# DigITs-AIML/MMNN_STS

Measured on AMD Instinct MI355X. Metric: training volumes/sec/GPU (128^3 T1+T2+preop, batch 2) at 1/2/4/8 MI355X, higher is better.
Workload: dtype f32; 1 GPU; configs[2] --images --preop --survival --blend: MultiModalModel(DenseNet121-3D(in=2), MLP(32), blend) fwd + GradientBlender Cox loss + bwd + grad all-reduce + SGD-Nesterov/OneCycle step, dropout 0.2; micro_batch=2, global_batch=2, tabular=32, parallelism=dp1, allreduce=none

## Files before the change

### mmnn_sts_amd/csrc/conv3_bf16x3.hip

```cpp
#include <stdlib.h>

#include "fprop.hpp"
#include "bf16x3.hpp"

namespace mmnn {

typedef float f32x16_t __attribute__((ext_vector_type(16)));
typedef __bf16 bf16x8_t __attribute__((ext_vector_type(8)));

namespace c3b {
constexpr int KC = 16, NT = 7, MAXC = 256;
template <int TD, int TH, int TW>
struct Geo {
  static constexpr int HD = TD + 2, HH = TH + 2, HW = TW + 2, HV = HD * HH * HW, ROWS = TD * TH * TW / 32;
  static constexpr int ITEMS = (2 * HV + 255) / 256;
  static constexpr size_t OPER_BYTES = (size_t)2 * 6 * HV * 16;
  static constexpr size_t SMEM = OPER_BYTES + sizeof(float) * (2 * 4 * 32 + 32);
  static_assert(TD * TH * TW % 32 == 0 && (TW == 32 || TW == 16), "rows of 32 voxels");
  static_assert(ITEMS <= NT, "one staging item per tap slot");
  static_assert(4 * ROWS * 16 * 64 * sizeof(float) <= OPER_BYTES, "the partial tiles are summed in the operand buffers");
  static_assert(SMEM <= 160 * 1024, "LDS");
};

__device__ __forceinline__ bf16x8_t as_bf16x8(uint4 v) { return __builtin_bit_cast(bf16x8_t, v); }
}

__global__ void __launch_bounds__(256) conv3_split_bnrelu_kernel(const FpropArgs a) {
  __shared__ float cf[2][8];
  const int c8 = blockIdx.y, n = blockIdx.z, C8 = a.Cin / 8, V = a.D * a.H * a.W;
  const int v = blockIdx.x * 256 + threadIdx.x;
  const float* __restrict__ x = a.in0 + (long)n * a.in0_ns + (long)(a.in0_coff + 8 * c8) * V;
  float xv[8];
#pragma unroll
  for (int e = 0; e < 8; ++e) xv[e] = v < V ? x[(long)e * V + v] : 0.f;
  if (threadIdx.x < 8) {
    float ca, cb, mu, rs;
    bn_fwd_coef(a.bn_in, 8 * c8 + threadIdx.x, ca, cb, mu, rs);
    cf[0][threadIdx.x] = ca; cf[1][threadIdx.x] = cb;
  }
  __syncthreads();
  if (v >= V) return;
#pragma unroll
  for (int e = 0; e < 8; ++e) xv[e] = fmaxf(fmaf(cf[0][e], xv[e], cf[1][e]), 0.f);
  uint4 hi, mid, lo;
  split3x8(xv, hi, mid, lo);
  const long ps = (long)a.N * C8 * V;
  uint4* __restrict__ dst = reinterpret_cast<uint4*>(a.x3) + ((long)n * C8 + c8) * V + v;
  dst[0] = hi; dst[ps] = mid; dst[2 * ps] = lo;
}

__global__ void __launch_bounds__(256) conv3_split_bnbwd_kernel(const FpropArgs a) {
  __shared__ float cf[3][8];
  const int c8 = blockIdx.y, n = blockIdx.z, C8 = a.Cin / 8, V = a.D * a.H * a.W;
  const int v = blockIdx.x * 256 + threadIdx.x;
  const float* __restrict__ gn = a.in0 + (long)n * a.in0_ns + (long)(a.in0_coff + 8 * c8) * V;
  const float* __restrict__ xn = a.in1 + (long)n * a.in1_ns + (long)(a.in1_coff + 8 * c8) * V;
  float gv[8], xv[8];
#pragma unroll
  for (int e = 0; e < 8; ++e) {
    gv[e] = v < V ? gn[(long)e * V + v] : 0.f;
    xv[e] = v < V ? xn[(long)e * V + v] : 0.f;
  }
  if (threadIdx.x < 8) {
    const int c = 8 * c8 + threadIdx.x;
    float p_, q_, r_;
    bn_bwd_coef(a.gr_in, c, p_, q_, r_);
    const float sc = drop_scale(a.drop_in, n, c);
    cf[0][threadIdx.x] = p_ * sc; cf[1][threadIdx.x] = q_ * sc; cf[2][threadIdx.x] = r_ * sc;
  }
  __syncthreads();
  if (v >= V) return;
#pragma unroll
  for (int e = 0; e < 8; ++e) gv[e] = fmaf(cf[0][e], gv[e], fmaf(cf[1][e], xv[e], cf[2][e]));
  uint4 hi, mid, lo;
  split3x8(gv, hi, mid, lo);
  const long ps = (long)a.N * C8 * V;
  uint4* __restrict__ dst = reinterpret_cast<uint4*>(a.x3) + ((long)n * C8 + c8) * V + v;
  dst[0] = hi; dst[ps] = mid; dst[2 * ps] = lo;
}

static int launch_split(bool bwd, const FpropArgs& a, hipStream_t stream) {
  const int V = a.D * a.H * a.W;
  const dim3 grid((unsigned)cdiv(V, 256), (unsigned)(a.Cin / 8), (unsigned)a.N);
  if (bwd) MMNN_LAUNCH(conv3_split_bnbwd_kernel, grid, dim3(256), 0, stream, a);
  else MMNN_LAUNCH(conv3_split_bnrelu_kernel, grid, dim3(256), 0, stream, a);
  MMNN_HIP(hipGetLastError());
  return 0;
}

template <int TD, int TH, int TW>
__global__ void __launch_bounds__(256) conv3_fwd_bf16x3_kernel(const FpropArgs a) {
  using namespace c3b;
  using G = Geo<TD, TH, TW>;
  constexpr int HH = G::HH, HW = G::HW, HV = G::HV, ROWS = G::ROWS, ITEMS = G::ITEMS;
  constexpr size_t OPER_BYTES = G::OPER_BYTES;
  extern __shared__ uint4 xs128[];
  float* const sred = reinterpret_cast<float*>(reinterpret_cast<char*>(xs128) + OPER_BYTES);
  float* const dsc = sred + 2 * 4 * 32;
  const int tid = threadIdx.x, lane = tid & 63, wv = tid >> 6;
  const int D = a.D, H = a.H, W = a.W, V = D * H * W, C8 = a.Cin / 8, nchunk = a.Cin / KC;
  const int twn = (W + TW - 1) / TW, thn = (H + TH - 1) / TH, tdn = (D + TD - 1) / TD;
  int b = blockIdx.x;
  const int w0 = (b % twn) * TW; b /= twn;
  const int h0 = (b % thn) * TH; b /= thn;
  const int d0 = (b % tdn) * TD;
  const int n = b / tdn;
  const long ps = (long)a.N * C8 * V;
  const uint4* __restrict__ xin = reinterpret_cast<const uint4*>(a.x3) + (long)n * C8 * V;
  const uint4* __restrict__ wp = reinterpret_cast<const uint4*>(a.w3);
  if (tid < 32) dsc[tid] = drop_scale(a.drop_out, n, tid);
  f32x16_t acc[ROWS];
#pragma unroll
  for (int t = 0; t < ROWS; ++t)
#pragma unroll
    for (int q = 0; q < 16; ++q) acc[t][q] = 0.f;
  uint4 xr[ITEMS][3];
  auto item_pos = [&](int it, int& g, int& hv, int& o) -> bool {
    const int item = tid + it * 256;
    g = item >= HV;
    hv = item - g * HV;
    const int hd = hv / (HH * HW), hh = (hv / HW) % HH, hw = hv % HW;
    const int d = d0 + hd - 1, h = h0 + hh - 1, w = w0 + hw - 1;
    o = (d * H + h) * W + w;
    return item < 2 * HV && (unsigned)d < (unsigned)D && (unsigned)h < (unsigned)H && (unsigned)w < (unsigned)W;
  };
  auto issue = [&](int ch) {
#pragma unroll
    for (int it = 0; it < ITEMS; ++it) {
      int g, hv, o;
      const bool ok = item_pos(it, g, hv, o);
      const uint4* src = xin + (long)(2 * ch + g) * V + o;
#pragma unroll
      for (int p = 0; p < 3; ++p) xr[it][p] = ok ? src[p * ps] : make_uint4(0u, 0u, 0u, 0u);
    }
  };
  auto commit_item = [&](int it, int buf) {
    int g, hv, o;
    item_pos(it, g, hv, o);
    if (tid + it * 256 >= 2 * HV) return;
    uint4* dst = xs128 + buf * (6 * HV);
#pragma unroll
    for (int p = 0; p < 3; ++p) dst[(p * 2 + g) * HV + hv] = xr[it][p];
  };
  bf16x8_t wr[NT][3];
  auto load_w = [&](int ti, int ch) {
    const int tap = wv + 4 * ti;
    if (tap < 27 && ch < nchunk) {
      const int c8 = 2 * ch + (lane >> 5);
#pragma unroll
      for (int p = 0; p < 3; ++p) wr[ti][p] = as_bf16x8(wp[((long)(p * 27 + tap) * C8 + c8) * 32 + (lane & 31)]);
    }
  };
#pragma unroll
  for (int ti = 0; ti < NT; ++ti) load_w(ti, 0);
  issue(0);
#pragma unroll
  for (int it = 0; it < ITEMS; ++it) commit_item(it, 0);
  __syncthreads();
  for (int ch = 0; ch < nchunk; ++ch) {
    const int cur = ch & 1;
    const bool more = ch + 1 < nchunk;
    if (more) issue(ch + 1);
#pragma unroll
    for (int ti = 0; ti < NT; ++ti) {
      const int tap = wv + 4 * ti;
      if (tap < 27) {
        const int td = tap / 9, th = (tap / 3) % 3, tw = tap % 3;
        bf16x8_t aw[3];
#pragma unroll
        for (int p = 0; p < 3; ++p) aw[p] = wr[ti][p];
        load_w(ti, ch + 1);
#pragma unroll
        for (int t = 0; t < ROWS; ++t) {
          const int v = t * 32 + (lane & 31);
          const int hv = ((v / (TW * TH) + td) * HH + ((v / TW) % TH + th)) * HW + (v % TW + tw);
          bf16x8_t bb[3];
#pragma unroll
          for (int p = 0; p < 3; ++p) bb[p] = as_bf16x8(xs128[cur * (6 * HV) + (p * 2 + (lane >> 5)) * HV + hv]);
          acc[t] = __builtin_amdgcn_mfma_f32_32x32x16_bf16(aw[1], bb[1], acc[t], 0, 0, 0);
          acc[t] = __builtin_amdgcn_mfma_f32_32x32x16_bf16(aw[0], bb[2], acc[t], 0, 0, 0);
          acc[t] = __builtin_amdgcn_mfma_f32_32x32x16_bf16(aw[2], bb[0], acc[t], 0, 0, 0);
          acc[t] = __builtin_amdgcn_mfma_f32_32x32x16_bf16(aw[0], bb[1], acc[t], 0, 0, 0);
          acc[t] = __builtin_amdgcn_mfma_f32_32x32x16_bf16(aw[1], bb[0], acc[t], 0, 0, 0);
          acc[t] = __builtin_amdgcn_mfma_f32_32x32x16_bf16(aw[0], bb[0], acc[t], 0, 0, 0);
        }
      }
      if (more && ti < ITEMS) commit_item(ti, cur ^ 1);
    }
    __syncthreads();
  }
  float* red = reinterpret_cast<float*>(xs128);
#pragma unroll
  for (int t = 0; t < ROWS; ++t)
#pragma unroll
    for (int q = 0; q < 16; ++q) red[((wv * ROWS + t) * 16 + q) * 64 + lane] = acc[t][q];
  __syncthreads();
  float* __restrict__ outn = a.out + (long)n * a.out_ns + (long)a.out_coff * V;
  const bool want_sums = a.st_out.sum != nullptr;
  float s0[16], s1[16];
#pragma unroll
  for (int q = 0; q < 16; ++q) { s0[q] = 0.f; s1[q] = 0.f; }
#pragma unroll
  for (int tt = 0; tt < (ROWS + 3) / 4; ++tt) {
    const int t = wv + 4 * tt;
    if (t >= ROWS) break;
    const int v = t * 32 + (lane & 31);
    const int d = d0 + v / (TW * TH), h = h0 + (v / TW) % TH, w = w0 + v % TW;
    const bool ok = d < D && h < H && w < W;
    const int o = (d * H + h) * W + w;
#pragma unroll
    for (int q = 0; q < 16; ++q) {
      float val = 0.f;
#pragma unroll
      for (int w2 = 0; w2 < 4; ++w2) val += red[((w2 * ROWS + t) * 16 + q) * 64 + lane];
      const int m = 8 * (q / 4) + 4 * (lane >> 5) + q % 4;
      val *= dsc[m];
      if (ok) {
        outn[(long)m * V + o] = val;
        s0[q] += val;
        s1[q] += val * val;
      }
    }
  }
  if (want_sums) {
#pragma unroll
    for (int q = 0; q < 16; ++q) {
      float t0 = s0[q], t1 = s1[q];
      t0 += swz_xor<16>(t0); t1 += swz_xor<16>(t1);
      t0 += swz_xor<8>(t0);  t1 += swz_xor<8>(t1);
      t0 += swz_xor<4>(t0);  t1 += swz_xor<4>(t1);
      t0 += swz_xor<2>(t0);  t1 += swz_xor<2>(t1);
      t0 += swz_xor<1>(t0);  t1 += swz_xor<1>(t1);
      if ((lane & 31) == 0) {
        const int m = 8 * (q / 4) + 4 * (lane >> 5) + q % 4;
        sred[wv * 32 + m] = t0;
        sred[4 * 32 + wv * 32 + m] = t1;
      }
    }
    __syncthreads();
    if (tid < 32) {
      const int rep = blockIdx.x & ((a.nrep > 0 ? a.nrep : NREP) - 1);
      double v0 = 0.0, v1 = 0.0;
#pragma unroll
      for (int w2 = 0; w2 < 4; ++w2) { v0 += (double)sred[w2 * 32 + tid]; v1 += (double)sred[4 * 32 + w2 * 32 + tid]; }
      atomicAdd(a.st_out.sum + (long)rep * a.st_out.stride + a.st_out.off + tid, v0);
      atomicAdd(a.st_out.sq + (long)rep * a.st_out.stride + a.st_out.off + tid, v1);
    }
  }
}

__global__ void __launch_bounds__(256) conv3_dgrad_bf16x3_kernel(const FpropArgs a) {
  using namespace c3b;
  using G = Geo<2, 4, 32>;
  constexpr int TH = 4, TW = 32, HH = G::HH, HW = G::HW, HV = G::HV, ROWS = G::ROWS, ITEMS = G::ITEMS, PF = 3, C8 = 4;
  extern __shared__ uint4 xs128[];
  float* const ecoef = reinterpret_cast<float*>(reinterpret_cast<char*>(xs128) + G::OPER_BYTES);
  const int tid = threadIdx.x, lane = tid & 63, wv = tid >> 6;
  const int D = a.D, H = a.H, W = a.W, V = D * H * W;
  const int twn = (W + TW - 1) / TW, thn = (H + TH - 1) / TH, tdn = (D + 1) / 2;
  int b = blockIdx.x;
  const int w0 = (b % twn) * TW; b /= twn;
  const int h0 = (b % thn) * TH; b /= thn;
  const int d0 = (b % tdn) * 2;
  const int n = b / tdn;
  const long ps = (long)a.N * C8 * V;
  const uint4* __restrict__ xin = reinterpret_cast<const uint4*>(a.x3) + (long)n * C8 * V;
  const uint4* __restrict__ wp = reinterpret_cast<const uint4*>(a.w3);
  uint4 xr[ITEMS][3];
  auto item_pos = [&](int it, int& g, int& hv, int& o) -> bool {
    const int item = tid + it * 256;
    g = item >= HV;
    hv = item - g * HV;
    const int hd = hv / (HH * HW), hh = (hv / HW) % HH, hw = hv % HW;
    const int d = d0 + hd - 1, h = h0 + hh - 1, w = w0 + hw - 1;
    o = (d * H + h) * W + w;
    return item < 2 * HV && (unsigned)d < (unsigned)D && (unsigned)h < (unsigned)H && (unsigned)w < (unsigned)W;
  };
  auto issue = [&](int ch) {
#pragma unroll
    for (int it = 0; it < ITEMS; ++it) {
      int g, hv, o;
      const bool ok = item_pos(it, g, hv, o);
      const uint4* src = xin + (long)(2 * ch + g) * V + o;
#pragma unroll
      for (int p = 0; p < 3; ++p) xr[it][p] = ok ? src[p * ps] : make_uint4(0u, 0u, 0u, 0u);
    }
  };
  auto commit = [&](int buf) {
#pragma unroll
    for (int it = 0; it < ITEMS; ++it) {
      int g, hv, o;
      item_pos(it, g, hv, o);
      if (tid + it * 256 < 2 * HV) {
        uint4* dst = xs128 + buf * (6 * HV);
#pragma unroll
        for (int p = 0; p < 3; ++p) dst[(p * 2 + g) * HV + hv] = xr[it][p];
      }
    }
  };
  bf16x8_t wr[PF][3];
  auto load_w = [&](int slot, int tap, int ch) {
    if (ch < 2) {
      const int c8 = 2 * ch + (lane >> 5);
#pragma unroll
      for (int p = 0; p < 3; ++p) wr[slot][p] = as_bf16x8(wp[((long)(p * 27 + tap) * C8 + c8) * 128 + wv * 32 + (lane & 31)]);
    }
  };
#pragma unroll
  for (int t = 0; t < PF; ++t) load_w(t, t, 0);
  issue(0);
  if (tid >= 128) {
    const int m = tid - 128;
    float ea, eb, mu, rs;
    bn_fwd_coef(a.ebn, m, ea, eb, mu, rs);
    ecoef[m] = ea; ecoef[128 + m] = eb; ecoef[256 + m] = mu; ecoef[384 + m] = rs;
  }
  commit(0);
  issue(1);
  __syncthreads();
  f32x16_t acc[ROWS];
#pragma unroll
  for (int t = 0; t < ROWS; ++t)
#pragma unroll
    for (int q = 0; q < 16; ++q) acc[t][q] = 0.f;
  auto pair = [&](int ch, int tq) {
    const int td = tq / 3, th = tq % 3;
#pragma unroll
    for (int tw = 0; tw < 3; ++tw) {
      const int tap = tq * 3 + tw;
      bf16x8_t aw[3];
#pragma unroll
      for (int p = 0; p < 3; ++p) aw[p] = wr[tw][p];
      if (tq < 8) load_w(tw, tap + PF, ch); else load_w(tw, tw, ch + 1);
#pragma unroll
      for (int t = 0; t < ROWS; ++t) {
        const int hv = ((t / TH + td) * HH + (t % TH + th)) * HW + ((lane & 31) + tw);
        bf16x8_t bb[3];
#pragma unroll
        for (int p = 0; p < 3; ++p) bb[p] = as_bf16x8(xs128[ch * (6 * HV) + (p * 2 + (lane >> 5)) * HV + hv]);
        acc[t] = __builtin_amdgcn_mfma_f32_32x32x16_bf16(aw[1], bb[1], acc[t], 0, 0, 0);
        acc[t] = __builtin_amdgcn_mfma_f32_32x32x16_bf16(aw[0], bb[2], acc[t], 0, 0, 0);
        acc[t] = __builtin_amdgcn_mfma_f32_32x32x16_bf16(aw[2], bb[0], acc[t], 0, 0, 0);
        acc[t] = __builtin_amdgcn_mfma_f32_32x32x16_bf16(aw[0], bb[1], acc[t], 0, 0, 0);
        acc[t] = __builtin_amdgcn_mfma_f32_32x32x16_bf16(aw[1], bb[0], acc[t], 0, 0, 0);
        acc[t] = __builtin_amdgcn_mfma_f32_32x32x16_bf16(aw[0], bb[0], acc[t], 0, 0, 0);
      }
    }
  };
  pair(0, 0);
  commit(1);
  __syncthreads();
#pragma unroll 1
  for (int tq = 1; tq < 9; ++tq) pair(0, tq);
#pragma unroll 1
  for (int tq = 0; tq < 9; ++tq) pair(1, tq);
  const float* __restrict__ exn = a.ex + (long)n * a.ex_ns + (long)a.ex_coff * V;
  float* __restrict__ outn = a.out + (long)n * a.out_ns + (long)a.out_coff * V;
  float s0[16], s1[16];
#pragma unroll
  for (int q = 0; q < 16; ++q) { s0[q] = 0.f; s1[q] = 0.f; }
  auto row_pos = [&](int t, int& o) -> bool {
    const int d = d0 + t / TH, h = h0 + t % TH, w = w0 + (lane & 31);
    o = (d * H + h) * W + w;
    return d < D && h < H && w < W;
  };
  float xn[16];
  {
    int o;
    const bool ok = row_pos(0, o);
#pragma unroll
    for (int q = 0; q < 16; ++q) xn[q] = ok ? exn[(long)(wv * 32 + 8 * (q / 4) + 4 * (lane >> 5) + q % 4) * V + o] : 0.f;
  }
#pragma unroll
  for (int t = 0; t < ROWS; ++t) {
    int o;
    const bool ok = row_pos(t, o);
    float xe[16];
#pragma unroll
    for (int q = 0; q < 16; ++q) xe[q] = xn[q];
    if (t + 1 < ROWS) {
      int o2;
      const bool ok2 = row_pos(t + 1, o2);
#pragma unroll
      for (int q = 0; q < 16; ++q) xn[q] = ok2 ? exn[(long)(wv * 32 + 8 * (q / 4) + 4 * (lane >> 5) + q % 4) * V + o2] : 0.f;
    }
#pragma unroll
    for (int q = 0; q < 16; ++q) {
      const int m = wv * 32 + 8 * (q / 4) + 4 * (lane >> 5) + q % 4;
      if (ok) {
        const float pre = fmaf(ecoef[m], xe[q], ecoef[128 + m]);
        const float z = pre > 0.f ? acc[t][q] : 0.f;
        const float xh = (xe[q] - ecoef[256 + m]) * ecoef[384 + m];
        outn[(long)m * V + o] = z;
        s0[q] += z;
        s1[q] += z * xh;
      }
    }
  }
  const int rep = blockIdx.x & ((a.nrep > 0 ? a.nrep : NREP) - 1);
#pragma unroll
  for (int q = 0; q < 16; ++q) {
    float t0 = s0[q], t1 = s1[q];
    t0 += swz_xor<16>(t0); t1 += swz_xor<16>(t1);
    t0 += swz_xor<8>(t0);  t1 += swz_xor<8>(t1);
    t0 += swz_xor<4>(t0);  t1 += swz_xor<4>(t1);
    t0 += swz_xor<2>(t0);  t1 += swz_xor<2>(t1);
    t0 += swz_xor<1>(t0);  t1 += swz_xor<1>(t1);
    if ((lane & 31) == 0) {
      const int m = wv * 32 + 8 * (q / 4) + 4 * (lane >> 5) + q % 4;
      atomicAdd(a.dbeta + (long)rep * a.M + m, (double)t0);
      atomicAdd(a.dgamma + (long)rep * a.M + m, (double)t1);
    }
  }
}

size_t conv3_bf16x3_plane_bytes(const FpropArgs& a) { return (size_t)3 * a.N * (a.Cin / 8) * a.D * a.H * a.W * 16; }

bool conv3_dgrad_bf16x3_eligible(const FpropArgs& a) {
  static const int mode = [] { const char* e = getenv("MMNN_BF16X3_DGRAD"); return e ? atoi(e) : 1; }();
  static const int fmode = [] { const char* e = getenv("MMNN_BF16X3"); return e ? atoi(e) : 32; }();
  return mode != 0 && fmode != 0 && a.M == 128 && a.Cin == 32 && a.W > 16;
}

int launch_conv3_dgrad_bf16x3(const FpropArgs& a, hipStream_t stream) {
  using G = c3b::Geo<2, 4, 32>;
  constexpr size_t SMEM = G::OPER_BYTES + sizeof(float) * 512;
  static_assert(SMEM <= 160 * 1024, "LDS");
  MMNN_REQUIRE(conv3_dgrad_bf16x3_eligible(a), "conv3 dgrad bf16x3: shape not handled (M=%d, Cin=%d, W=%d)", a.M, a.Cin, a.W);
  MMNN_REQUIRE(a.in1 && a.ex && a.dgamma && a.dbeta, "conv3 dgrad bf16x3: operands missing");
  MMNN_REQUIRE(a.w3 && a.x3 && a.x3_bytes >= conv3_bf16x3_plane_bytes(a), "conv3 dgrad bf16x3: pre-split weights or plane scratch missing");
  MMNN_REQUIRE((long)(a.M + 1) * a.D * a.H * a.W < (1l << 31), "conv3 dgrad bf16x3: volume too large for 32-bit element offsets");
  const long tiles = (long)a.N * cdiv(a.D, 2) * cdiv(a.H, 4) * cdiv(a.W, 32);
  MMNN_REQUIRE(tiles > 0 && tiles < (1l << 31), "conv3 dgrad bf16x3: grid out of range");
  static bool configured[MAX_DEVICES] = {false};
  bool& conf = configured[current_device_slot()];
  if (!conf) {
    MMNN_HIP(hipFuncSetAttribute(reinterpret_cast<const void*>(conv3_dgrad_bf16x3_kernel), hipFuncAttributeMaxDynamicSharedMemorySize, (int)SMEM));
    conf = true;
  }
  if (int rc = launch_split(true, a, stream)) return rc;
  MMNN_LAUNCH(conv3_dgrad_bf16x3_kernel, dim3((unsigned)tiles), dim3(256), SMEM, stream, a);
  MMNN_HIP(hipGetLastError());
  return 0;
}

bool conv3_fwd_bf16x3_eligible(const FpropArgs& a) {
  static const int mode = [] { const char* e = getenv("MMNN_BF16X3"); return e ? atoi(e) : 32; }();
  return mode != 0 && a.M == 32 && a.Cin % c3b::KC == 0 && a.Cin >= c3b::KC && a.Cin <= c3b::MAXC && a.W > 16;
}

int launch_conv3_fwd_bf16x3(const FpropArgs& a, hipStream_t stream) {
  using G = c3b::Geo<2, 4, 32>;
  MMNN_REQUIRE(conv3_fwd_bf16x3_eligible(a), "conv3 bf16x3: shape not handled (M=%d, Cin=%d, W=%d)", a.M, a.Cin, a.W);
  MMNN_REQUIRE(a.drop_in.p <= 0.f, "conv3 bf16x3: no input dropout on this path");
  MMNN_REQUIRE(a.w3 && a.x3 && a.x3_bytes >= conv3_bf16x3_plane_bytes(a), "conv3 bf16x3: pre-split weights or plane scratch missing");
  MMNN_REQUIRE((long)(a.Cin + 1) * a.D * a.H * a.W < (1l << 31), "conv3 bf16x3: volume too large for 32-bit element offsets");
  const long tiles = (long)a.N * cdiv(a.D, 2) * cdiv(a.H, 4) * cdiv(a.W, 32);
  MMNN_REQUIRE(tiles > 0 && tiles < (1l << 31), "conv3 bf16x3: grid out of range");
  static bool configured[MAX_DEVICES] = {false};
  bool& conf = configured[current_device_slot()];
  if (!conf) {
    MMNN_HIP(hipFuncSetAttribute(reinterpret_cast<const void*>(conv3_fwd_bf16x3_kernel<2, 4, 32>), hipFuncAttributeMaxDynamicSharedMemorySize, (int)G::SMEM));
    conf = true;
  }
  if (int rc = launch_split(false, a, stream)) return rc;
  MMNN_LAUNCH((conv3_fwd_bf16x3_kernel<2, 4, 32>), dim3((unsigned)tiles), dim3(256), G::SMEM, stream, a);
  MMNN_HIP(hipGetLastError());
  return 0;
}

}
```

### mmnn_sts_amd/csrc/densenet.hip

```cpp
#include "densenet.hpp"

#include <string.h>

#include <algorithm>

#include "fprop.hpp"
#include "stem.hpp"
#include "wgrad.hpp"

namespace mmnn {

static size_t align_up(size_t v, size_t a = 256) { return (v + a - 1) / a * a; }
constexpr size_t KZ_PART_BYTES = (size_t)512 * 4 * 1024 * sizeof(float);
constexpr unsigned KZ_CNT_ENTRIES = 4096;

namespace {
struct Panel { const float* p; unsigned bytes; };
struct Carver {
  size_t cur = 0;
  size_t take(size_t bytes) {
    size_t o = cur;
    cur = align_up(cur + bytes);
    return o;
  }
// ... 55 lines not shown
      bn(p.mid, lo.n2w, lo.n2b, lo.r2m, lo.r2v);
      lo.c2 = po; po += conv2_elems(p);
      p.layers[b].push_back(lo);
      ci += cfg.growth;
    }
    if (b != cfg.nblocks - 1) {
      TransOff t;
      t.cin = ci; t.cout = ci / 2;
      bn(ci, t.nw, t.nb, t.rm, t.rv);
      t.cw = po; po += trans_elems(t);
      p.trans.push_back(t);
    } else {
      bn(ci, p.p_n5w, p.p_n5b, p.r_n5m, p.r_n5v);
    }
  }
  p.n_params = po; p.n_runstats = ro; p.n_bn = nbn;

  Carver cv;
  const int nb = cfg.nblocks;
  const size_t F = sizeof(float);
  const long V0 = (long)p.D0 * p.H0 * p.W0;
  p.o_conv0 = cv.take((size_t)N * cfg.init_features * V0 * F);
  p.o_idx = cv.take((size_t)N * cfg.init_features * p.Vb[0]);
  p.o_t1.assign(nb, {});
  size_t dap = 0;
  for (int b = 0; b < nb; ++b) {
    p.o_x[b] = cv.take((size_t)N * p.ctot_b[b] * p.Vb[b] * F);
    p.o_g[b] = cv.take((size_t)N * p.ctot_b[b] * p.Vb[b] * F);
    for (int l = 0; l < cfg.block_layers[b]; ++l) p.o_t1[b].push_back(cv.take((size_t)N * p.mid * p.Vb[b] * F));
    if (b != nb - 1) {
      p.o_ap[b] = cv.take((size_t)N * p.ctot_b[b] * p.Vb[b + 1] * F);
      dap = std::max(dap, (size_t)N * p.ctot_b[b] * p.Vb[b + 1] * F);
    } else {
      p.o_ap[b] = 0;
    }
  }
  p.o_dap = cv.take(dap ? dap : 256);
  p.o_dz0 = cv.take((size_t)N * cfg.init_features * V0 * F);
  const size_t PAIR = 2 * NREP * sizeof(double);
  p.o_fstat = cv.cur;
  p.o_st_conv0 = cv.take(PAIR * cfg.init_features);
  p.o_st_t1.assign(nb, {});
  for (int b = 0; b < nb; ++b) {
    p.o_st_x[b] = cv.take(PAIR * p.ctot_b[b]);
    for (int l = 0; l < cfg.block_layers[b]; ++l) p.o_st_t1[b].push_back(cv.take(PAIR * p.mid));
  }
  p.fstat_bytes = cv.cur - p.o_fstat;
  p.o_bstat = cv.cur;
  p.o_dg_n0 = cv.take(PAIR * cfg.init_features);
  p.o_dg_n1.assign(nb, {}); p.o_dg_n2.assign(nb, {}); p.o_dg_tr.clear();
  for (int b = 0; b < nb; ++b) {
    p.o_s_x[b] = cv.take(PAIR * p.ctot_b[b]);
    for (int l = 0; l < cfg.block_layers[b]; ++l) {
      p.o_dg_n1[b].push_back(cv.take(PAIR * p.layers[b][l].cin));
      p.o_dg_n2[b].push_back(cv.take(PAIR * p.mid));
    }
    if (b != nb - 1) p.o_dg_tr.push_back(cv.take(PAIR * p.ctot_b[b]));
  }
  p.o_dg_n5 = cv.take(PAIR * p.ctot_b[nb - 1]);
  p.bstat_bytes = cv.cur - p.o_bstat;
  p.o_pk_conv0 = cv.take((size_t)7 * stem_krows(cfg.in_channels) * 64 * F);
  p.o_pk_c1.assign(nb, {}); p.o_pk_c2f.assign(nb, {}); p.o_pk_c2b.assign(nb, {}); p.o_pk_tr.clear();
  p.o_pk_c2f3.assign(nb, {}); p.o_pk_c2b3.assign(nb, {});
  p.x3_bytes = 0;
  for (int b = 0; b < nb; ++b) {
    FpropArgs f, g;
    memset(&f, 0, sizeof(f));
    f.N = N; f.D = p.Db[b]; f.H = p.Hb[b]; f.W = p.Wb[b];
    g = f;
    f.Cin = p.mid; f.M = cfg.growth;
    g.Cin = cfg.growth; g.M = p.mid;
    const bool f3 = conv3_fwd_bf16x3_eligible(f), b3 = conv3_dgrad_bf16x3_eligible(g);
    if (f3) p.x3_bytes = std::max(p.x3_bytes, conv3_bf16x3_plane_bytes(f));
    if (b3) p.x3_bytes = std::max(p.x3_bytes, conv3_bf16x3_plane_bytes(g));
    for (int l = 0; l < cfg.block_layers[b]; ++l) {
      p.o_pk_c1[b].push_back(cv.take(conv1_elems(p, p.layers[b][l].cin) * F));
      p.o_pk_c2f[b].push_back(cv.take(conv2_elems(p) * F));
      p.o_pk_c2b[b].push_back(cv.take(conv2_elems(p) * F));
      p.o_pk_c2f3[b].push_back(f3 ? cv.take(conv2_split_bytes(p)) : 0);
      p.o_pk_c2b3[b].push_back(b3 ? cv.take(conv2_split_bytes(p)) : 0);
    }
    if (b != nb - 1) p.o_pk_tr.push_back(cv.take(trans_elems(p.trans[b]) * F));
  }
  p.o_x3 = p.x3_bytes ? cv.take(p.x3_bytes) : 0;
  p.ns_conv0 = stem_wgrad_pick_splits(N, p.D0, p.H0, p.W0, cfg.in_channels);
  p.o_sl_conv0 = cv.take((size_t)p.ns_conv0 * cfg.in_channels * cfg.init_features * 352 * F);
  p.o_sl_c1.assign(nb, {}); p.o_sl_c2.assign(nb, {}); p.ns_c1.assign(nb, {}); p.ns_c2.assign(nb, {});
  p.o_sl_tr.clear(); p.ns_tr.clear();
  for (int b = 0; b < nb; ++b) {
    for (int l = 0; l < cfg.block_layers[b]; ++l) {
      const int ci = p.layers[b][l].cin;
      int pairs = 0;
      {
        const int cw = wgrad1_channel_width(ci, p.Vb[b]);
        for (int k = 0; k < cfg.block_layers[b]; ++k)
          if (wgrad1_channel_width(p.layers[b][k].cin, p.Vb[b]) == cw) pairs += cdiv(p.layers[b][k].cin, cw);
      }
      const int s1 = wgrad_pick_splits(1, N, p.Db[b], p.Hb[b], p.Wb[b], p.mid, ci, pairs);
      const int s2 = wgrad_pick_splits(27, N, p.Db[b], p.Hb[b], p.Wb[b], cfg.growth, p.mid, cfg.block_layers[b]);
      p.ns_c1[b].push_back(s1); p.ns_c2[b].push_back(s2);
      p.o_sl_c1[b].push_back(cv.take(s1 * conv1_elems(p, ci) * F));
      p.o_sl_c2[b].push_back(cv.take(s2 * conv2_elems(p) * F));
    }
    if (b != nb - 1) {
      const int s = wgrad_pick_splits(1, N, p.Db[b + 1], p.Hb[b + 1], p.Wb[b + 1], p.trans[b].cout, p.trans[b].cin);
      p.ns_tr.push_back(s);
      p.o_sl_tr.push_back(cv.take(s * trans_elems(p.trans[b]) * F));
    }
  }
  for (int b = 0; b < nb; ++b) p.o_dz2[b] = cv.take((size_t)cfg.block_layers[b] * N * p.mid * p.Vb[b] * F);
  p.o_kz_part = cv.take(KZ_PART_BYTES);
  p.o_kz_cnt = cv.take(KZ_CNT_ENTRIES * sizeof(unsigned));
  int nlayers = 0;
  for (int b = 0; b < nb; ++b) nlayers += cfg.block_layers[b];
  p.n_run_jobs = nbn;
  p.n_pack_jobs = 1 + 5 * nlayers + (nb - 1);
  p.n_grad_jobs = 3 + 6 * nlayers + 3 * (nb - 1) + 2;
  p.o_jobs_run = cv.take(sizeof(RunStatJob) * p.n_run_jobs);
  p.o_jobs_pack = cv.take(sizeof(PackJob) * p.n_pack_jobs);
  p.o_jobs_grad = cv.take(sizeof(GradJob) * p.n_grad_jobs);
  p.n_layers = nlayers;
  p.o_wg_table = cv.take(sizeof(WgradArgs) * 2 * nlayers);
  p.ws_bytes = cv.cur;
  p.host_jobs_bytes = p.o_wg_table - p.o_jobs_run;
  if (p.host_jobs) { (void)hipHostFree(p.host_jobs); p.host_jobs = nullptr; }
  p.tab_params = nullptr; p.tab_run = nullptr; p.tab_ws = nullptr;
  return 0;
}

void plan_free(Plan& p) {
  if (p.host_jobs) (void)hipHostFree(p.host_jobs);
  p.host_jobs = nullptr;
  if (p.wg_pinned) (void)hipHostFree(p.wg_pinned);
  p.wg_pinned = nullptr;
  for (hipEvent_t e : p.timer_ev) (void)hipEventDestroy(e);
  p.timer_ev.clear();
}

static NormSite concat_site(const Plan& p, int b, int C, long w, long bb, long rm, long rv, size_t o_dg) {
  return {p.o_st_x[b], p.o_s_x[b], o_dg, p.ctot_b[b], 0, C, p.nrep_b[b], w, bb, rm, rv, (double)p.N * p.Vb[b]};
}
static NormSite norm0(const Plan& p) {
  const int C = p.cfg.init_features;
  return {p.o_st_conv0, p.o_dg_n0, p.o_dg_n0, C, 0, C, NREP, p.p_n0w, p.p_n0b, p.r_n0m, p.r_n0v, (double)p.N * p.D0 * p.H0 * p.W0};
}
static NormSite norm1(const Plan& p, int b, int l) {
  const LayerOff& lo = p.layers[b][l];
  return concat_site(p, b, lo.cin, lo.n1w, lo.n1b, lo.r1m, lo.r1v, p.o_dg_n1[b][l]);
}
static NormSite norm2(const Plan& p, int b, int l) {
  const LayerOff& lo = p.layers[b][l];
  return {p.o_st_t1[b][l], p.o_dg_n2[b][l], p.o_dg_n2[b][l], p.mid, 0, p.mid, p.nrep_b[b], lo.n2w, lo.n2b, lo.r2m, lo.r2v, (double)p.N * p.Vb[b]};
}
static NormSite transition(const Plan& p, int b) {
  const TransOff& t = p.trans[b];
  return concat_site(p, b, t.cin, t.nw, t.nb, t.rm, t.rv, p.o_dg_tr[b]);
}
static NormSite norm5(const Plan& p) {
  const int b = p.cfg.nblocks - 1;
  return concat_site(p, b, p.ctot_b[b], p.p_n5w, p.p_n5b, p.r_n5m, p.r_n5v, p.o_dg_n5);
}

static StatPtr statptr(char* ws, size_t o, int C, int off, int nrep) {
  StatPtr s; memset(&s, 0, sizeof(s));
  s.sum = reinterpret_cast<double*>(ws + o); s.sq = s.sum + (long)NREP * C;
  s.stride = C; s.off = off; s.nrep = nrep;
  return s;
// ... 552 lines not shown
```

Before: 260.5 volumes/s (whole job; 1 volume = 1 patient = stacked T1+T2 2x128^3 + 32 tabular).

## Stage conv3 bf16x3 halo tiles via direct global-to-LDS loads interleaved with MFMAs

Replaces the register-staged halo loads in the 3x3x3 bf16x3 forward and dgrad kernels with global_load_lds_dwordx4 copies that write straight into LDS. Out-of-bounds voxels are pointed at a zero entry placed just past the plane scratch, which the split kernels write. The copies are spread through the MFMA loop, and LDS operand fetches are double-buffered one row ahead under sched_barriers. The aim is to cut VGPR pressure and staging latency so loads overlap with tensor-core work. In exchange it depends on inline asm that sets m0, a padded halo layout, and a one-entry scratch over-allocation.

```diff
diff --git a/mmnn_sts_amd/csrc/conv3_bf16x3.hip b/mmnn_sts_amd/csrc/conv3_bf16x3.hip
--- a/mmnn_sts_amd/csrc/conv3_bf16x3.hip
+++ b/mmnn_sts_amd/csrc/conv3_bf16x3.hip
@@ -2,6 +2,7 @@
 
 #include "fprop.hpp"
 #include "bf16x3.hpp"
+#include "conv3_stage_map.hpp"
 
 namespace mmnn {
 
@@ -13,16 +14,29 @@
 template <int TD, int TH, int TW>
 struct Geo {
   static constexpr int HD = TD + 2, HH = TH + 2, HW = TW + 2, HV = HD * HH * HW, ROWS = TD * TH * TW / 32;
-  static constexpr int ITEMS = (2 * HV + 255) / 256;
-  static constexpr size_t OPER_BYTES = (size_t)2 * 6 * HV * 16;
+  static constexpr int PPP = c3map::Halo<TD, TH, TW>::PPP, HVP = c3map::Halo<TD, TH, TW>::HVP;
+  static constexpr size_t OPER_BYTES = (size_t)2 * 6 * HVP * 16;
   static constexpr size_t SMEM = OPER_BYTES + sizeof(float) * (2 * 4 * 32 + 32);
   static_assert(TD * TH * TW % 32 == 0 && (TW == 32 || TW == 16), "rows of 32 voxels");
-  static_assert(ITEMS <= NT, "one staging item per tap slot");
+  static_assert(PPP <= 16, "a wave stages at most four piece columns");
   static_assert(4 * ROWS * 16 * 64 * sizeof(float) <= OPER_BYTES, "the partial tiles are summed in the operand buffers");
   static_assert(SMEM <= 160 * 1024, "LDS");
 };
 
 __device__ __forceinline__ bf16x8_t as_bf16x8(uint4 v) { return __builtin_bit_cast(bf16x8_t, v); }
+
+__device__ __forceinline__ void glds16(const uint4* src, uint4* lds) {
+  const unsigned dst = __builtin_amdgcn_readfirstlane((unsigned)(size_t)(__attribute__((address_space(3))) void*)lds);
+  unsigned keep;
+  asm volatile("s_mov_b32 %0, m0\n\ts_mov_b32 m0, %2\n\ts_nop 0\n\tglobal_load_lds_dwordx4 %1, off\n\ts_mov_b32 m0, %0"
+               : "=&s"(keep) : "v"(src), "s"(dst) : "memory");
+}
+__device__ __forceinline__ void dma_wait_all() { asm volatile("s_waitcnt vmcnt(0)" ::: "memory"); }
+}
+
+__device__ __forceinline__ void write_zero_entry(const FpropArgs& a) {
+  if ((blockIdx.x | blockIdx.y | blockIdx.z | threadIdx.x) == 0)
+    *reinterpret_cast<uint4*>(static_cast<char*>(a.x3) + a.x3_bytes) = make_uint4(0u, 0u, 0u, 0u);
 }
 
 __global__ void __launch_bounds__(256) conv3_split_bnrelu_kernel(const FpropArgs a) {
@@ -33,6 +47,7 @@
   float xv[8];
 #pragma unroll
   for (int e = 0; e < 8; ++e) xv[e] = v < V ? x[(long)e * V + v] : 0.f;
+  write_zero_entry(a);
   if (threadIdx.x < 8) {
     float ca, cb, mu, rs;
     bn_fwd_coef(a.bn_in, 8 * c8 + threadIdx.x, ca, cb, mu, rs);
@@ -61,6 +76,7 @@
     gv[e] = v < V ? gn[(long)e * V + v] : 0.f;
     xv[e] = v < V ? xn[(long)e * V + v] : 0.f;
   }
+  write_zero_entry(a);
   if (threadIdx.x < 8) {
     const int c = 8 * c8 + threadIdx.x;
     float p_, q_, r_;
@@ -92,12 +108,12 @@
 __global__ void __launch_bounds__(256) conv3_fwd_bf16x3_kernel(const FpropArgs a) {
   using namespace c3b;
   using G = Geo<TD, TH, TW>;
-  constexpr int HH = G::HH, HW = G::HW, HV = G::HV, ROWS = G::ROWS, ITEMS = G::ITEMS;
+  constexpr int HH = G::HH, HW = G::HW, HVP = G::HVP, PPP = G::PPP, ROWS = G::ROWS;
   constexpr size_t OPER_BYTES = G::OPER_BYTES;
   extern __shared__ uint4 xs128[];
   float* const sred = reinterpret_cast<float*>(reinterpret_cast<char*>(xs128) + OPER_BYTES);
   float* const dsc = sred + 2 * 4 * 32;
-  const int tid = threadIdx.x, lane = tid & 63, wv = tid >> 6;
+  const int tid = threadIdx.x, lane = tid & 63, wv = __builtin_amdgcn_readfirstlane(tid >> 6);
   const int D = a.D, H = a.H, W = a.W, V = D * H * W, C8 = a.Cin / 8, nchunk = a.Cin / KC;
   const int twn = (W + TW - 1) / TW, thn = (H + TH - 1) / TH, tdn = (D + TD - 1) / TD;
   int b = blockIdx.x;
@@ -105,88 +121,95 @@
   const int h0 = (b % thn) * TH; b /= thn;
   const int d0 = (b % tdn) * TD;
   const int n = b / tdn;
-  const long ps = (long)a.N * C8 * V;
-  const uint4* __restrict__ xin = reinterpret_cast<const uint4*>(a.x3) + (long)n * C8 * V;
+  const uint4* __restrict__ x3 = reinterpret_cast<const uint4*>(a.x3);
   const uint4* __restrict__ wp = reinterpret_cast<const uint4*>(a.w3);
+  const long zero_entry = (long)(a.x3_bytes / 16);
   if (tid < 32) dsc[tid] = drop_scale(a.drop_out, n, tid);
   f32x16_t acc[ROWS];
 #pragma unroll
   for (int t = 0; t < ROWS; ++t)
 #pragma unroll
     for (int q = 0; q < 16; ++q) acc[t][q] = 0.f;
-  uint4 xr[ITEMS][3];
-  auto item_pos = [&](int it, int& g, int& hv, int& o) -> bool {
-    const int item = tid + it * 256;
-    g = item >= HV;
-    hv = item - g * HV;
-    const int hd = hv / (HH * HW), hh = (hv / HW) % HH, hw = hv % HW;
-    const int d = d0 + hd - 1, h = h0 + hh - 1, w = w0 + hw - 1;
-    o = (d * H + h) * W + w;
-    return item < 2 * HV && (unsigned)d < (unsigned)D && (unsigned)h < (unsigned)H && (unsigned)w < (unsigned)W;
-  };
-  auto issue = [&](int ch) {
-#pragma unroll
-    for (int it = 0; it < ITEMS; ++it) {
-      int g, hv, o;
-      const bool ok = item_pos(it, g, hv, o);
-      const uint4* src = xin + (long)(2 * ch + g) * V + o;
-#pragma unroll
-      for (int p = 0; p < 3; ++p) xr[it][p] = ok ? src[p * ps] : make_uint4(0u, 0u, 0u, 0u);
-    }
-  };
-  auto commit_item = [&](int it, int buf) {
-    int g, hv, o;
-    item_pos(it, g, hv, o);
-    if (tid + it * 256 >= 2 * HV) return;
-    uint4* dst = xs128 + buf * (6 * HV);
-#pragma unroll
-    for (int p = 0; p < 3; ++p) dst[(p * 2 + g) * HV + hv] = xr[it][p];
+  const int j0 = c3map::wave_col<TD, TH, TW>(3, wv, 0);
+  int so[4];
+#pragma unroll
+  for (int i = 0; i < 4; ++i) {
+    const int col = c3map::wave_col<TD, TH, TW>(3, wv, i);
+    so[i] = col >= 0 ? c3map::halo_voxel<TD, TH, TW>(col * 64 + lane, d0, h0, w0, D, H, W) : -1;
+  }
+  static_assert(PPP == 13, "three waves x three columns + one wave x four");
+  auto stage = [&](int q, int ch, int buf, bool live) {
+    const int i = q / 6, plane = q % 6;
+    glds16(x3 + c3map::src_entry(plane, live ? so[i] : -1, ch, n, a.N, C8, V, zero_entry), xs128 + buf * (6 * HVP) + plane * HVP + (j0 + 4 * i) * 64);
   };
   bf16x8_t wr[NT][3];
   auto load_w = [&](int ti, int ch) {
     const int tap = wv + 4 * ti;
-    if (tap < 27 && ch < nchunk) {
-      const int c8 = 2 * ch + (lane >> 5);
+    if (tap < 27) {
+      const int c8 = 2 * min(ch, nchunk - 1) + (lane >> 5);
 #pragma unroll
       for (int p = 0; p < 3; ++p) wr[ti][p] = as_bf16x8(wp[((long)(p * 27 + tap) * C8 + c8) * 32 + (lane & 31)]);
     }
   };
 #pragma unroll
+  for (int q = 0; q < 18; ++q) stage(q, 0, 0, true);
+  if (wv == 3) {
+#pragma unroll
+    for (int q = 18; q < 24; ++q) stage(q, 0, 0, true);
+  }
+#pragma unroll
   for (int ti = 0; ti < NT; ++ti) load_w(ti, 0);
-  issue(0);
-#pragma unroll
-  for (int it = 0; it < ITEMS; ++it) commit_item(it, 0);
+  const int lrow = (lane >> 5) * HVP + (lane & 31);
+  auto tap_off = [&](int ti) {
+    const int tap = min(wv + 4 * ti, 26);
+    return ((tap / 9) * HH + (tap / 3) % 3) * HW + tap % 3;
+  };
+  auto fetch = [&](bf16x8_t (&bb)[3], int cur, int toff, int t) {
+    const uint4* src = xs128 + cur * (6 * HVP) + lrow + toff + ((t / TH) * HH + t % TH) * HW;
+#pragma unroll
+    for (int p = 0; p < 3; ++p) bb[p] = as_bf16x8(src[p * 2 * HVP]);
+  };
+  bf16x8_t bb[2][3];
+  dma_wait_all();
   __syncthreads();
   for (int ch = 0; ch < nchunk; ++ch) {
     const int cur = ch & 1;
     const bool more = ch + 1 < nchunk;
-    if (more) issue(ch + 1);
+    int toff = tap_off(0);
+#pragma unroll
+    for (int t = 0; t < ROWS; ++t) asm volatile("" : "+a"(acc[t]));
+    fetch(bb[0], cur, toff, 0);
 #pragma unroll
     for (int ti = 0; ti < NT; ++ti) {
       const int tap = wv + 4 * ti;
-      if (tap < 27) {
-        const int td = tap / 9, th = (tap / 3) % 3, tw = tap % 3;
+      const int toffn = ti + 1 < NT ? tap_off(ti + 1) : 0;
+      if (ti < NT - 1 || tap < 27) {
         bf16x8_t aw[3];
 #pragma unroll
         for (int p = 0; p < 3; ++p) aw[p] = wr[ti][p];
         load_w(ti, ch + 1);
 #pragma unroll
         for (int t = 0; t < ROWS; ++t) {
-          const int v = t * 32 + (lane & 31);
-          const int hv = ((v / (TW * TH) + td) * HH + ((v / TW) % TH + th)) * HW + (v % TW + tw);
-          bf16x8_t bb[3];
-#pragma unroll
-          for (int p = 0; p < 3; ++p) bb[p] = as_bf16x8(xs128[cur * (6 * HV) + (p * 2 + (lane >> 5)) * HV + hv]);
-          acc[t] = __builtin_amdgcn_mfma_f32_32x32x16_bf16(aw[1], bb[1], acc[t], 0, 0, 0);
-          acc[t] = __builtin_amdgcn_mfma_f32_32x32x16_bf16(aw[0], bb[2], acc[t], 0, 0, 0);
-          acc[t] = __builtin_amdgcn_mfma_f32_32x32x16_bf16(aw[2], bb[0], acc[t], 0, 0, 0);
-          acc[t] = __builtin_amdgcn_mfma_f32_32x32x16_bf16(aw[0], bb[1], acc[t], 0, 0, 0);
-          acc[t] = __builtin_amdgcn_mfma_f32_32x32x16_bf16(aw[1], bb[0], acc[t], 0, 0, 0);
-          acc[t] = __builtin_amdgcn_mfma_f32_32x32x16_bf16(aw[0], bb[0], acc[t], 0, 0, 0);
+          const int s = (ti * ROWS + t) & 1;
+          if (t + 1 < ROWS) fetch(bb[s ^ 1], cur, toff, t + 1);
+          else if (ti + 1 < NT) fetch(bb[s ^ 1], cur, toffn, 0);
+          __builtin_amdgcn_sched_barrier(0);
+          acc[t] = __builtin_amdgcn_mfma_f32_32x32x16_bf16(aw[1], bb[s][1], acc[t], 0, 0, 0);
+          acc[t] = __builtin_amdgcn_mfma_f32_32x32x16_bf16(aw[0], bb[s][2], acc[t], 0, 0, 0);
+          acc[t] = __builtin_amdgcn_mfma_f32_32x32x16_bf16(aw[2], bb[s][0], acc[t], 0, 0, 0);
+          acc[t] = __builtin_amdgcn_mfma_f32_32x32x16_bf16(aw[0], bb[s][1], acc[t], 0, 0, 0);
+          acc[t] = __builtin_amdgcn_mfma_f32_32x32x16_bf16(aw[1], bb[s][0], acc[t], 0, 0, 0);
+          acc[t] = __builtin_amdgcn_mfma_f32_32x32x16_bf16(aw[0], bb[s][0], acc[t], 0, 0, 0);
+          if (ti < 6 && t % 2 == 1 && t < 6) stage(3 * ti + t / 2, ch + 1, cur ^ 1, more);
+          __builtin_amdgcn_sched_barrier(0);
         }
+      } else {
+#pragma unroll
+        for (int q = 18; q < 24; ++q) stage(q, ch + 1, cur ^ 1, more);
       }
-      if (more && ti < ITEMS) commit_item(ti, cur ^ 1);
-    }
+      toff = toffn;
+    }
+    dma_wait_all();
     __syncthreads();
   }
   float* red = reinterpret_cast<float*>(xs128);
@@ -252,10 +275,10 @@
 __global__ void __launch_bounds__(256) conv3_dgrad_bf16x3_kernel(const FpropArgs a) {
   using namespace c3b;
   using G = Geo<2, 4, 32>;
-  constexpr int TH = 4, TW = 32, HH = G::HH, HW = G::HW, HV = G::HV, ROWS = G::ROWS, ITEMS = G::ITEMS, PF = 3, C8 = 4;
+  constexpr int TH = 4, TW = 32, HH = G::HH, HW = G::HW, HVP = G::HVP, PPP = G::PPP, ROWS = G::ROWS, PF = 3, C8 = 4;
   extern __shared__ uint4 xs128[];
   float* const ecoef = reinterpret_cast<float*>(reinterpret_cast<char*>(xs128) + G::OPER_BYTES);
-  const int tid = threadIdx.x, lane = tid & 63, wv = tid >> 6;
+  const int tid = threadIdx.x, lane = tid & 63, wv = __builtin_amdgcn_readfirstlane(tid >> 6);
   const int D = a.D, H = a.H, W = a.W, V = D * H * W;
   const int twn = (W + TW - 1) / TW, thn = (H + TH - 1) / TH, tdn = (D + 1) / 2;
   int b = blockIdx.x;
@@ -263,97 +286,98 @@
   const int h0 = (b % thn) * TH; b /= thn;
   const int d0 = (b % tdn) * 2;
   const int n = b / tdn;
-  const long ps = (long)a.N * C8 * V;
-  const uint4* __restrict__ xin = reinterpret_cast<const uint4*>(a.x3) + (long)n * C8 * V;
+  const uint4* __restrict__ x3 = reinterpret_cast<const uint4*>(a.x3);
   const uint4* __restrict__ wp = reinterpret_cast<const uint4*>(a.w3);
-  uint4 xr[ITEMS][3];
-  auto item_pos = [&](int it, int& g, int& hv, int& o) -> bool {
-    const int item = tid + it * 256;
-    g = item >= HV;
-    hv = item - g * HV;
-    const int hd = hv / (HH * HW), hh = (hv / HW) % HH, hw = hv % HW;
-    const int d = d0 + hd - 1, h = h0 + hh - 1, w = w0 + hw - 1;
-    o = (d * H + h) * W + w;
-    return item < 2 * HV && (unsigned)d < (unsigned)D && (unsigned)h < (unsigned)H && (unsigned)w < (unsigned)W;
-  };
-  auto issue = [&](int ch) {
-#pragma unroll
-    for (int it = 0; it < ITEMS; ++it) {
-      int g, hv, o;
-      const bool ok = item_pos(it, g, hv, o);
-      const uint4* src = xin + (long)(2 * ch + g) * V + o;
-#pragma unroll
-      for (int p = 0; p < 3; ++p) xr[it][p] = ok ? src[p * ps] : make_uint4(0u, 0u, 0u, 0u);
-    }
-  };
-  auto commit = [&](int buf) {
-#pragma unroll
-    for (int it = 0; it < ITEMS; ++it) {
-      int g, hv, o;
-      item_pos(it, g, hv, o);
-      if (tid + it * 256 < 2 * HV) {
-        uint4* dst = xs128 + buf * (6 * HV);
-#pragma unroll
-        for (int p = 0; p < 3; ++p) dst[(p * 2 + g) * HV + hv] = xr[it][p];
-      }
-    }
+  const long zero_entry = (long)(a.x3_bytes / 16);
+  int so[4];
+#pragma unroll
+  for (int i = 0; i < 4; ++i) {
+    const int col = c3map::wave_col<2, TH, TW>(0, wv, i);
+    so[i] = col >= 0 ? c3map::halo_voxel<2, TH, TW>(col * 64 + lane, d0, h0, w0, D, H, W) : -1;
+  }
+  static_assert(PPP == 13, "four columns in wave 0, three in the others");
+  auto stage = [&](int q, int ch) {
+    const int i = q / 6, plane = q % 6;
+    glds16(x3 + c3map::src_entry(plane, so[i], ch, n, a.N, C8, V, zero_entry), xs128 + ch * (6 * HVP) + plane * HVP + (wv + 4 * i) * 64);
   };
   bf16x8_t wr[PF][3];
   auto load_w = [&](int slot, int tap, int ch) {
-    if (ch < 2) {
-      const int c8 = 2 * ch + (lane >> 5);
-#pragma unroll
-      for (int p = 0; p < 3; ++p) wr[slot][p] = as_bf16x8(wp[((long)(p * 27 + tap) * C8 + c8) * 128 + wv * 32 + (lane & 31)]);
-    }
-  };
+    const int c8 = 2 * ch + (lane >> 5);
+#pragma unroll
+    for (int p = 0; p < 3; ++p) wr[slot][p] = as_bf16x8(wp[((long)(p * 27 + tap) * C8 + c8) * 128 + wv * 32 + (lane & 31)]);
+  };
+#pragma unroll
+  for (int q = 0; q < 18; ++q) stage(q, 0);
+  if (wv == 0) {
+#pragma unroll
+    for (int q = 18; q < 24; ++q) stage(q, 0);
+  }
 #pragma unroll
   for (int t = 0; t < PF; ++t) load_w(t, t, 0);
-  issue(0);
   if (tid >= 128) {
     const int m = tid - 128;
     float ea, eb, mu, rs;
     bn_fwd_coef(a.ebn, m, ea, eb, mu, rs);
     ecoef[m] = ea; ecoef[128 + m] = eb; ecoef[256 + m] = mu; ecoef[384 + m] = rs;
   }
-  commit(0);
-  issue(1);
+  dma_wait_all();
   __syncthreads();
   f32x16_t acc[ROWS];
 #pragma unroll
   for (int t = 0; t < ROWS; ++t)
 #pragma unroll
     for (int q = 0; q < 16; ++q) acc[t][q] = 0.f;
-  auto pair = [&](int ch, int tq) {
-    const int td = tq / 3, th = tq % 3;
+  const int lrow = (lane >> 5) * HVP + (lane & 31);
+  auto pair_off = [&](int pi) {
+    const int ch = pi / 9, tq = pi % 9;
+    return ch * (6 * HVP) + ((tq / 3) * HH + tq % 3) * HW;
+  };
+  auto fetch = [&](bf16x8_t (&bb)[3], int poff, int tw, int t) {
+    const uint4* src = xs128 + lrow + poff + ((t / TH) * HH + t % TH) * HW + tw;
+#pragma unroll
+    for (int p = 0; p < 3; ++p) bb[p] = as_bf16x8(src[p * 2 * HVP]);
+  };
+  bf16x8_t bb[2][3];
+  auto pair = [&](int pi, bool first) {
+    const int ch = pi / 9, tq = pi % 9;
+    const int poff = pair_off(pi), poffn = pair_off(min(pi + 1, 17));
 #pragma unroll
     for (int tw = 0; tw < 3; ++tw) {
       const int tap = tq * 3 + tw;
       bf16x8_t aw[3];
 #pragma unroll
       for (int p = 0; p < 3; ++p) aw[p] = wr[tw][p];
-      if (tq < 8) load_w(tw, tap + PF, ch); else load_w(tw, tw, ch + 1);
+      load_w(tw, tq < 8 ? tap + PF : tw, tq < 8 ? ch : 1);
 #pragma unroll
       for (int t = 0; t < ROWS; ++t) {
-        const int hv = ((t / TH + td) * HH + (t % TH + th)) * HW + ((lane & 31) + tw);
-        bf16x8_t bb[3];
-#pragma unroll
-        for (int p = 0; p < 3; ++p) bb[p] = as_bf16x8(xs128[ch * (6 * HV) + (p * 2 + (lane >> 5)) * HV + hv]);
-        acc[t] = __builtin_amdgcn_mfma_f32_32x32x16_bf16(aw[1], bb[1], acc[t], 0, 0, 0);
-        acc[t] = __builtin_amdgcn_mfma_f32_32x32x16_bf16(aw[0], bb[2], acc[t], 0, 0, 0);
-        acc[t] = __builtin_amdgcn_mfma_f32_32x32x16_bf16(aw[2], bb[0], acc[t], 0, 0, 0);
-        acc[t] = __builtin_amdgcn_mfma_f32_32x32x16_bf16(aw[0], bb[1], acc[t], 0, 0, 0);
-        acc[t] = __builtin_amdgcn_mfma_f32_32x32x16_bf16(aw[1], bb[0], acc[t], 0, 0, 0);
-        acc[t] = __builtin_amdgcn_mfma_f32_32x32x16_bf16(aw[0], bb[0], acc[t], 0, 0, 0);
+        const int s = t & 1;
+        if (t + 1 < ROWS) fetch(bb[s ^ 1], poff, tw, t + 1);
+        else if (tw < 2) fetch(bb[s ^ 1], poff, tw + 1, 0);
+        else if (!first) fetch(bb[s ^ 1], poffn, 0, 0);
+        __builtin_amdgcn_sched_barrier(0);
+        acc[t] = __builtin_amdgcn_mfma_f32_32x32x16_bf16(aw[1], bb[s][1], acc[t], 0, 0, 0);
+        acc[t] = __builtin_amdgcn_mfma_f32_32x32x16_bf16(aw[0], bb[s][2], acc[t], 0, 0, 0);
+        acc[t] = __builtin_amdgcn_mfma_f32_32x32x16_bf16(aw[2], bb[s][0], acc[t], 0, 0, 0);
+        acc[t] = __builtin_amdgcn_mfma_f32_32x32x16_bf16(aw[0], bb[s][1], acc[t], 0, 0, 0);
+        acc[t] = __builtin_amdgcn_mfma_f32_32x32x16_bf16(aw[1], bb[s][0], acc[t], 0, 0, 0);
+        acc[t] = __builtin_amdgcn_mfma_f32_32x32x16_bf16(aw[0], bb[s][0], acc[t], 0, 0, 0);
+        if (first && 8 * tw + t < 18) stage(8 * tw + t, 1);
+        __builtin_amdgcn_sched_barrier(0);
       }
     }
-  };
-  pair(0, 0);
-  commit(1);
-  __syncthreads();
+    if (first && wv == 0) {
+#pragma unroll
+      for (int q = 18; q < 24; ++q) stage(q, 1);
+    }
+  };
+  fetch(bb[0], pair_off(0), 0, 0);
+  pair(0, true);
+  dma_wait_all();
+  __syncthreads();
+  fetch(bb[0], pair_off(1), 0, 0);
 #pragma unroll 1
-  for (int tq = 1; tq < 9; ++tq) pair(0, tq);
-#pragma unroll 1
-  for (int tq = 0; tq < 9; ++tq) pair(1, tq);
+  for (int pi = 1; pi < 17; ++pi) pair(pi, false);
+  constexpr int EP = 3;
   const float* __restrict__ exn = a.ex + (long)n * a.ex_ns + (long)a.ex_coff * V;
   float* __restrict__ outn = a.out + (long)n * a.out_ns + (long)a.out_coff * V;
   float s0[16], s1[16];
@@ -364,26 +388,24 @@
     o = (d * H + h) * W + w;
     return d < D && h < H && w < W;
   };
-  float xn[16];
-  {
+  float xr[EP][16];
+  auto load_row = [&](int t) {
     int o;
-    const bool ok = row_pos(0, o);
-#pragma unroll
-    for (int q = 0; q < 16; ++q) xn[q] = ok ? exn[(long)(wv * 32 + 8 * (q / 4) + 4 * (lane >> 5) + q % 4) * V + o] : 0.f;
-  }
+    const bool ok = row_pos(t, o);
+#pragma unroll
+    for (int q = 0; q < 16; ++q) xr[t % EP][q] = ok ? exn[(long)(wv * 32 + 8 * (q / 4) + 4 * (lane >> 5) + q % 4) * V + o] : 0.f;
+  };
+#pragma unroll
+  for (int t = 0; t < EP; ++t) load_row(t);
+  pair(17, false);
 #pragma unroll
   for (int t = 0; t < ROWS; ++t) {
     int o;
     const bool ok = row_pos(t, o);
     float xe[16];
 #pragma unroll
-    for (int q = 0; q < 16; ++q) xe[q] = xn[q];
-    if (t + 1 < ROWS) {
-      int o2;
-      const bool ok2 = row_pos(t + 1, o2);
-#pragma unroll
-      for (int q = 0; q < 16; ++q) xn[q] = ok2 ? exn[(long)(wv * 32 + 8 * (q / 4) + 4 * (lane >> 5) + q % 4) * V + o2] : 0.f;
-    }
+    for (int q = 0; q < 16; ++q) xe[q] = xr[t % EP][q];
+    if (t + EP < ROWS) load_row(t + EP);
 #pragma unroll
     for (int q = 0; q < 16; ++q) {
       const int m = wv * 32 + 8 * (q / 4) + 4 * (lane >> 5) + q % 4;
@@ -428,7 +450,7 @@
   static_assert(SMEM <= 160 * 1024, "LDS");
   MMNN_REQUIRE(conv3_dgrad_bf16x3_eligible(a), "conv3 dgrad bf16x3: shape not handled (M=%d, Cin=%d, W=%d)", a.M, a.Cin, a.W);
   MMNN_REQUIRE(a.in1 && a.ex && a.dgamma && a.dbeta, "conv3 dgrad bf16x3: operands missing");
-  MMNN_REQUIRE(a.w3 && a.x3 && a.x3_bytes >= conv3_bf16x3_plane_bytes(a), "conv3 dgrad bf16x3: pre-split weights or plane scratch missing");
+  MMNN_REQUIRE(a.w3 && a.x3 && a.x3_bytes % 16 == 0 && a.x3_bytes >= conv3_bf16x3_plane_bytes(a), "conv3 dgrad bf16x3: pre-split weights or plane scratch missing");
   MMNN_REQUIRE((long)(a.M + 1) * a.D * a.H * a.W < (1l << 31), "conv3 dgrad bf16x3: volume too large for 32-bit element offsets");
   const long tiles = (long)a.N * cdiv(a.D, 2) * cdiv(a.H, 4) * cdiv(a.W, 32);
   MMNN_REQUIRE(tiles > 0 && tiles < (1l << 31), "conv3 dgrad bf16x3: grid out of range");
@@ -453,7 +475,7 @@
   using G = c3b::Geo<2, 4, 32>;
   MMNN_REQUIRE(conv3_fwd_bf16x3_eligible(a), "conv3 bf16x3: shape not handled (M=%d, Cin=%d, W=%d)", a.M, a.Cin, a.W);
   MMNN_REQUIRE(a.drop_in.p <= 0.f, "conv3 bf16x3: no input dropout on this path");
-  MMNN_REQUIRE(a.w3 && a.x3 && a.x3_bytes >= conv3_bf16x3_plane_bytes(a), "conv3 bf16x3: pre-split weights or plane scratch missing");
+  MMNN_REQUIRE(a.w3 && a.x3 && a.x3_bytes % 16 == 0 && a.x3_bytes >= conv3_bf16x3_plane_bytes(a), "conv3 bf16x3: pre-split weights or plane scratch missing");
   MMNN_REQUIRE((long)(a.Cin + 1) * a.D * a.H * a.W < (1l << 31), "conv3 bf16x3: volume too large for 32-bit element offsets");
   const long tiles = (long)a.N * cdiv(a.D, 2) * cdiv(a.H, 4) * cdiv(a.W, 32);
   MMNN_REQUIRE(tiles > 0 && tiles < (1l << 31), "conv3 bf16x3: grid out of range");
diff --git a/mmnn_sts_amd/csrc/conv3_stage_map.hpp b/mmnn_sts_amd/csrc/conv3_stage_map.hpp
--- /dev/null
+++ b/mmnn_sts_amd/csrc/conv3_stage_map.hpp
@@ -0,0 +1,50 @@
+#pragma once
+
+#if defined(__HIPCC__) || defined(__CUDACC__)
+#define C3MAP_HD __host__ __device__
+#else
+#define C3MAP_HD
+#endif
+
+namespace mmnn {
+namespace c3map {
+
+template <int TD, int TH, int TW>
+struct Halo {
+  static constexpr int HD = TD + 2, HH = TH + 2, HW = TW + 2, HV = HD * HH * HW;
+  static constexpr int PPP = (HV + 63) / 64;
+  static constexpr int HVP = PPP * 64;
+  static constexpr int PIECES = 6 * PPP;
+};
+
+template <int TD, int TH, int TW>
+C3MAP_HD inline int halo_voxel(int e, int d0, int h0, int w0, int D, int H, int W) {
+  using G = Halo<TD, TH, TW>;
+  if (e >= G::HV) return -1;
+  const int hd = e / (G::HH * G::HW), hh = (e / G::HW) % G::HH, hw = e % G::HW;
+  const int d = d0 + hd - 1, h = h0 + hh - 1, w = w0 + hw - 1;
+  const bool in = (unsigned)d < (unsigned)D && (unsigned)h < (unsigned)H && (unsigned)w < (unsigned)W;
+  return in ? (d * H + h) * W + w : -1;
+}
+
+C3MAP_HD inline long src_entry(int plane, int vox, int ch, int n, int N, int C8, int V, long zero_entry) {
+  if (vox < 0) return zero_entry;
+  const int piece = plane >> 1, c8 = 2 * ch + (plane & 1);
+  return ((long)piece * N + n) * C8 * V + (long)c8 * V + vox;
+}
+
+template <int TD, int TH, int TW>
+C3MAP_HD inline int wave_col(int w4, int wv, int i) {
+  const int col = ((wv - w4) & 3) + 4 * i;
+  return col < Halo<TD, TH, TW>::PPP ? col : -1;
+}
+
+template <int TD, int TH, int TW>
+C3MAP_HD inline long stage_src(int s, int lane, int ch, int n, int d0, int h0, int w0, int N, int C8, int D, int H, int W, long zero_entry) {
+  using G = Halo<TD, TH, TW>;
+  const int plane = s / G::PPP, col = s % G::PPP;
+  return src_entry(plane, halo_voxel<TD, TH, TW>(col * 64 + lane, d0, h0, w0, D, H, W), ch, n, N, C8, D * H * W, zero_entry);
+}
+
+}
+}
diff --git a/mmnn_sts_amd/csrc/densenet.hip b/mmnn_sts_amd/csrc/densenet.hip
--- a/mmnn_sts_amd/csrc/densenet.hip
+++ b/mmnn_sts_amd/csrc/densenet.hip
@@ -161,7 +161,7 @@
     }
     if (b != nb - 1) p.o_pk_tr.push_back(cv.take(trans_elems(p.trans[b]) * F));
   }
-  p.o_x3 = p.x3_bytes ? cv.take(p.x3_bytes) : 0;
+  p.o_x3 = p.x3_bytes ? cv.take(p.x3_bytes + 16) : 0;
   p.ns_conv0 = stem_wgrad_pick_splits(N, p.D0, p.H0, p.W0, cfg.in_channels);
   p.o_sl_conv0 = cv.take((size_t)p.ns_conv0 * cfg.in_channels * cfg.init_features * 352 * F);
   p.o_sl_c1.assign(nb, {}); p.o_sl_c2.assign(nb, {}); p.ns_c1.assign(nb, {}); p.ns_c2.assign(nb, {});
```

New measurement: 260.6 volumes/s (whole job; 1 volume = 1 patient = stacked T1+T2 2x128^3 + 32 tabular) (median of 5 runs). About the same (+0.0%).
